# strukturag/libheif

Hardware: NVIDIA H100
Metric: megapixels/sec HEIC-grid decode->RGB (higher is better)
Workload: dtype u8

## Files before the change

libheif_b200/csrc/b200_hevc_entropy.cu:

```cuda
#include <cstdint>
#include <cstdlib>
namespace b200 { namespace syn {
__shared__ uint32_t s_kLps4[64];
__shared__ uint8_t s_kTransLps[64];
__shared__ uint8_t s_kNextState[256];
__shared__ unsigned long long s_kState[128];
__shared__ uint8_t s_kInitI[135];
__shared__ uint8_t s_kSigMap4[16];
__shared__ uint8_t s_kScanPos[3][16];
__shared__ uint8_t s_kScanInv[3][16];
__shared__ uint8_t s_kSbInv[4][3][64];
__shared__ uint8_t s_kSigCtx4[3][16];
__shared__ uint8_t s_kSigCtxN[3][4][16];
__shared__ uint8_t s_kChromaTab[4];
__shared__ uint8_t s_kScanX[4][3][64];
__shared__ uint8_t s_kScanY[4][3][64];
} }
#ifdef __CUDA_ARCH__
#define B200_T(name) s_##name
#endif
#include "b200_hevc.h"
static_assert(b200::syn::CTX_COUNT == 135, "s_kInitI above is sized for 135 context variables");

namespace b200 {

#ifndef B200_ENTROPY_WARPS
#define B200_ENTROPY_WARPS 4
#endif
constexpr int EWARPS = B200_ENTROPY_WARPS;

__device__ __forceinline__ unsigned e_ld_acquire(const unsigned* p) {
  unsigned v; asm volatile("ld.relaxed.gpu.global.u32 %0, [%1];" : "=r"(v) : "l"(p) : "memory"); return v;
}
__device__ __forceinline__ void e_st_release(unsigned* p, unsigned v) {
  asm volatile("st.release.gpu.global.u32 [%0], %1;" ::"l"(p), "r"(v) : "memory");
}
__device__ __forceinline__ unsigned e_poll(const unsigned* p) { return __shfl_sync(0xffffffffu, e_ld_acquire(p), 0); }
__device__ __forceinline__ bool lane0() { return syn::lane_id() == 0; }

#ifdef B200_ENTROPY_TRACE
constexpr int TRACE_CAP = 1 << 16;
__device__ unsigned long long g_trace[TRACE_CAP][2];
__device__ unsigned g_trace_sm[TRACE_CAP];
__device__ __forceinline__ unsigned long long e_globaltimer() { unsigned long long t; asm volatile("mov.u64 %0, %%globaltimer;" : "=l"(t)); return t; }
__device__ __forceinline__ unsigned e_smid() { unsigned s; asm volatile("mov.u32 %0, %%smid;" : "=r"(s)); return s; }
#endif

struct DevSync {
  unsigned* progress;
  unsigned* sub_done;
  unsigned* error_flag;
  unsigned* queue; unsigned* qtail; unsigned* deps;
  uint32_t dense_tu, dense_coef, dense_tu_cap, dense_coef_cap;
  uint64_t end_bit_position;
  __device__ static void spin_until(const unsigned* p, unsigned need, unsigned* error_flag) {
    if (e_poll(p) >= need) return;
    unsigned ns = 200, spins = 0;
    for (;;) {
      __nanosleep(ns); if (ns < 8000) ns <<= 1;
      if (e_poll(p) >= need) return;
      if ((++spins & 63u) != 0) continue;
      if (e_poll(error_flag)) return;
      if (spins > (1u << 23)) { if (lane0()) atomicExch(error_flag, 3u); return; }
    }
  }
  __device__ void wait_row(int row, int need) { spin_until(progress + row, (unsigned)need, error_flag); }
  __device__ void publish_row(int row, int done) { syn::warp_sync(); if (lane0()) e_st_release(progress + row, (unsigned)done); }
  __device__ void wait_substream(int idx) { spin_until(sub_done + idx, 1u, error_flag); }
  __device__ void finish_substream(int idx, int err) {
    syn::warp_sync();
    if (lane0()) {
      e_st_release(sub_done + idx, 1u);
      if (err) atomicExch(error_flag, (unsigned)err);
    }
  }
  __device__ void notify(int target) {
    if (target < 0) return;
    syn::warp_sync();
    if (lane0()) {
      __threadfence();
      if (atomicSub(deps + target, 1u) == 1u) { const unsigned s = atomicAdd(qtail, 1u); e_st_release(queue + s, (unsigned)target + 1u); }
    }
  }
};

#ifndef B200_ENTROPY_MIN_BLOCKS
#define B200_ENTROPY_MIN_BLOCKS 1
#endif
#ifndef B200_ENTROPY_MAX_BLOCKS_PER_SM
#define B200_ENTROPY_MAX_BLOCKS_PER_SM 0
#endif
template <class Cfg> constexpr int entropy_min_blocks() { return B200_ENTROPY_MIN_BLOCKS; }
template <> constexpr int entropy_min_blocks<syn::CfgCommon>() { return B200_ENTROPY_MIN_BLOCKS > 5 ? B200_ENTROPY_MIN_BLOCKS : 5; }
template <class Cfg>
__global__ void __launch_bounds__(EWARPS * 32, entropy_min_blocks<Cfg>()) hevc_entropy_kernel(const EntropyBatch b) {
  __shared__ __align__(8) syn::U2 s_ctx[EWARPS][syn::CTX_COUNT + syn::CTX_SCRATCH];
  __shared__ syn::DecoderT<Cfg> s_dec[EWARPS];
  __shared__ DevSync s_sync[EWARPS];
  for (int i = threadIdx.x; i < 64; i += blockDim.x) { syn::s_kLps4[i] = syn::d_kLps4[i]; syn::s_kTransLps[i] = syn::d_kTransLps[i]; }
  for (int i = threadIdx.x; i < syn::CTX_COUNT; i += blockDim.x) syn::s_kInitI[i] = syn::d_kInitI[i];
  for (int i = threadIdx.x; i < 256; i += blockDim.x) syn::s_kNextState[i] = syn::d_kNextState[i];
  for (int i = threadIdx.x; i < 128; i += blockDim.x) syn::s_kState[i] = syn::d_kState[i];
  for (int i = threadIdx.x; i < 16; i += blockDim.x) syn::s_kSigMap4[i] = syn::d_kSigMap4[i];
  for (int i = threadIdx.x; i < 48; i += blockDim.x) { (&syn::s_kScanPos[0][0])[i] = (&syn::d_kScanPos[0][0])[i]; (&syn::s_kScanInv[0][0])[i] = (&syn::d_kScanInv[0][0])[i]; (&syn::s_kSigCtx4[0][0])[i] = (&syn::d_kSigCtx4[0][0])[i]; }
  for (int i = threadIdx.x; i < 192; i += blockDim.x) (&syn::s_kSigCtxN[0][0][0])[i] = (&syn::d_kSigCtxN[0][0][0])[i];
  for (int i = threadIdx.x; i < 768; i += blockDim.x) (&syn::s_kSbInv[0][0][0])[i] = (&syn::d_kSbInv[0][0][0])[i];
  for (int i = threadIdx.x; i < 4; i += blockDim.x) syn::s_kChromaTab[i] = syn::d_kChromaTab[i];
  for (int i = threadIdx.x; i < 4 * 3 * 64; i += blockDim.x) { (&syn::s_kScanX[0][0][0])[i] = (&syn::d_kScanX[0][0][0])[i]; (&syn::s_kScanY[0][0][0])[i] = (&syn::d_kScanY[0][0][0])[i]; }
  __syncthreads();
  const int slot_w = threadIdx.x >> 5;
  const syn::CtxPtr ctx = (syn::CtxPtr)__cvta_generic_to_shared(s_ctx[slot_w]);
  for (;;) {
    unsigned slot = 0;
    if (lane0()) slot = atomicAdd(b.qhead, 1u);
    slot = __shfl_sync(0xffffffffu, slot, 0);
    if (slot >= (unsigned)b.nsubs) break;
    unsigned item = e_poll(b.queue + slot);
    if (!item) {
      unsigned ns = 500, spins = 0;
      for (;;) {
        __nanosleep(ns); if (ns < 16000) ns <<= 1;
        if ((item = e_poll(b.queue + slot)) != 0u) break;
        if ((++spins & 31u) != 0) continue;
        if (e_poll(b.error_flag)) return;
        if (spins > (1u << 22)) { if (lane0()) atomicExch(b.error_flag, 3u); return; }
      }
    }
#ifdef B200_ENTROPY_TRACE
    if (lane0() && item - 1u < (unsigned)TRACE_CAP) { g_trace[item - 1u][0] = e_globaltimer(); g_trace_sm[item - 1u] = e_smid(); }
#endif
    const syn::Substream& gs = b.subs[item - 1u];
    const EntropyPic& ep = b.pics[gs.pic];
    DevSync& sync = s_sync[slot_w];
    sync.progress = b.progress + ep.progress_base; sync.sub_done = b.sub_done + ep.sub_base; sync.error_flag = b.error_flag;
    sync.queue = b.queue; sync.qtail = b.qtail; sync.deps = b.deps;
    sync.dense_tu = sync.dense_coef = sync.dense_tu_cap = sync.dense_coef_cap = 0; sync.end_bit_position = 0;
    syn::run_substream<Cfg>(s_dec[slot_w], ep.sp, ep.pb, b.subs + ep.sub_base, (int)(item - 1u - ep.sub_base), ctx, sync);
#ifdef B200_ENTROPY_TRACE
    if (lane0() && item - 1u < (unsigned)TRACE_CAP) g_trace[item - 1u][1] = e_globaltimer();
#endif
  }
}

#ifdef B200_ENTROPY_TRACE
extern "C" int b200_debug_entropy_trace(unsigned long long* out, int n) {
  if (!out || n < 0 || n > TRACE_CAP) return set_error(B200_E_INVALID, "bad trace request");
  static unsigned long long t[TRACE_CAP][2]; static unsigned sm[TRACE_CAP];
  cudaError_t e = cudaDeviceSynchronize();
  if (e == cudaSuccess) e = cudaMemcpyFromSymbol(t, g_trace, sizeof t);
  if (e == cudaSuccess) e = cudaMemcpyFromSymbol(sm, g_trace_sm, sizeof sm);
  if (e != cudaSuccess) return set_error(B200_E_CUDA, "entropy trace: %s", cudaGetErrorString(e));
  for (int i = 0; i < n; i++) { out[3 * i] = t[i][0]; out[3 * i + 1] = t[i][1]; out[3 * i + 2] = sm[i]; }
  return B200_OK;
}
#endif
// ... 65 lines not shown
```

libheif_b200/csrc/b200_hevc_syntax.h:

```cpp
#pragma once
#include <cassert>
#include <cstdint>
#include <cstring>
#include "b200_hevc_types.h"

#if defined(__CUDA_ARCH__) && !defined(B200_SYNTAX_HOST_ONLY)
#define B200_SYN_DEVICE 1
#endif
#if defined(__CUDACC__) && !defined(B200_SYNTAX_HOST_ONLY)
#define B200_HDN __host__ __device__ __noinline__
#define B200_NOUNROLL _Pragma("unroll 1")
#define B200_HD __host__ __device__
#define B200_HDI __host__ __device__ __forceinline__
#define B200_TABLE(type, name, dims, ...) static const type h_##name dims = __VA_ARGS__; static __device__ const type d_##name dims = __VA_ARGS__;
#else
#define B200_HDN
#define B200_NOUNROLL
#define B200_HD
#define B200_HDI inline
#define B200_TABLE(type, name, dims, ...) static const type h_##name dims = __VA_ARGS__;
#endif
#if defined(B200_SYN_DEVICE) && !defined(B200_T)
#define B200_T(name) d_##name
#endif
// ... 84 lines not shown
#define B200_LANES_BEGIN() assert(__activemask() == 0xffffffffu)
#else
#define B200_LANES_BEGIN() ((void)0)
#endif
#define B200_LANE_FOR(k, n) B200_NOUNROLL for (int k = ::b200::syn::lane_id(); k < (n); k += 32)
#define B200_LANES_END() ::b200::syn::warp_sync()
#else
#define B200_LANES_BEGIN() ((void)0)
#define B200_LANE_FOR(k, n) B200_NOUNROLL for (int k = 0; k < (n); k++)
#define B200_LANES_END() ((void)0)
#endif

struct SeqParams {
  int32_t W, H, log2ctb, wctb, hctb, w4, w8, h8, chroma, bd;
  int32_t log2_min_cb, log2_min_tb, log2_max_tb, max_th_depth_intra;
  int32_t sao_enabled, transform_skip, cu_qp_delta, qg_log2, sign_hiding, wpp, sao_scale_luma, sao_scale_chroma;
  int32_t dense;
  int32_t tu_slots, coef_slots;
  int32_t pcm, pcm_bd_y, pcm_bd_c, pcm_shift_y, pcm_shift_c, log2_min_pcm, log2_max_pcm, pcm_lf_disabled;
  int32_t tq_bypass;
  int32_t tiles;
};

struct Substream {
  uint32_t pic;
  uint32_t byte_begin, byte_end;
  uint32_t ctb_begin, ctb_end;
  uint16_t tile_x0, tile_x1;
  uint32_t slice_addr_rs;
  int32_t slice_idx;
  int32_t slice_qp;
  uint8_t sao_luma, sao_chroma;
  uint8_t init_contexts;
  uint8_t last_of_segment;
  int32_t prev;
  int32_t wake_ctb2;
  int32_t wake_end;
  uint32_t deps;
};

struct PicBuffers {
  const uint8_t* rbsp; uint32_t rbsp_size;
  TuCmd* tus; CoefEntry* coefs; CtuInfo* ctus; const SliceInfo* slices;
  const uint16_t* ctu_slice;
  int8_t* qp8; uint8_t* edge8;
  uint8_t* ipm4;
  uint8_t* cd8;
  uint8_t* wpp_ctx;
  uint8_t* end_state;
};

B200_TABLE(uint8_t, kNextState, [256], {2,3,4,5,6,7,8,9,10,11,12,13,14,15,16,17,18,19,20,21,22,23,24,25,26,27,28,29,30,31,32,33,34,35,36,37,38,39,40,41,42,43,44,45,46,47,48,49,50,51,52,53,54,55,56,57,58,59,60,61,62,63,64,65,66,67,68,69,70,71,72,73,74,75,76,77,78,79,80,81,82,83,84,85,86,87,88,89,90,91,92,93,94,95,96,97,98,99,100,101,102,103,104,105,106,107,108,109,110,111,112,113,114,115,116,117,118,119,120,121,122,123,124,125,124,125,126,127,1,0,0,1,2,3,4,5,4,5,8,9,8,9,10,11,12,13,14,15,16,17,18,19,18,19,22,23,22,23,24,25,26,27,26,27,30,31,30,31,32,33,32,33,36,37,36,37,38,39,38,39,42,43,42,43,44,45,44,45,46,47,48,49,48,49,50,51,52,53,52,53,54,55,54,55,56,57,58,59,58,59,60,61,60,61,60,61,62,63,64,65,64,65,66,67,66,67,66,67,68,69,68,69,70,71,70,71,70,71,72,73,72,73,72,73,74,75,74,75,74,75,76,77,76,77,126,127})

B200_TABLE(uint64_t, kState, [128], {0x00000102f0d0b080ull,0x01000003f0d0b080ull,0x02000004e3c5a780ull,0x03000105e3c5a780ull,0x04000206d8bb9e80ull,0x05000307d8bb9e80ull,0x06000408cdb2967bull,0x07000509cdb2967bull,0x0800040ac3a98e74ull,0x0900050bc3a98e74ull,0x0a00080cb9a0876full,0x0b00090db9a0876full,0x0c00080eaf988069ull,0x0d00090faf988069ull,0x0e000a10a6907a64ull,0x0f000b11a6907a64ull,0x10000c129e89745full,0x11000d139e89745full,0x12000e1496826e5aull,0x13000f1596826e5aull,0x140010168e7b6855ull,0x150011178e7b6855ull,0x1600121887756351ull,0x1700131987756351ull,0x1800121a806f5e4dull,0x1900131b806f5e4dull,0x1a00161c7a695949ull,0x1b00171d7a695949ull,0x1c00161e74645545ull,0x1d00171f74645545ull,0x1e0018206e5f5042ull,0x1f0019216e5f5042ull,0x20001a22685a4c3eull,0x21001b23685a4c3eull,0x22001a246356483bull,0x23001b256356483bull,0x24001e265e514538ull,0x25001f275e514538ull,0x26001e28594d4135ull,0x27001f29594d4135ull,0x2800202a55493e33ull,0x2900212b55493e33ull,0x2a00202c50453b30ull,0x2b00212d50453b30ull,0x2c00242e4c42382eull,0x2d00252f4c42382eull,0x2e002430483f352bull,0x2f002531483f352bull,0x30002632453b3229ull,0x31002733453b3229ull,0x3200263441383027ull,0x3300273541383027ull,0x34002a363e362d25ull,0x35002b373e362d25ull,0x36002a383b332b23ull,0x37002b393b332b23ull,0x38002c3a38302921ull,0x39002d3b38302921ull,0x3a002c3c352e2720ull,0x3b002d3d352e2720ull,0x3c002e3e322b251eull,0x3d002f3f322b251eull,0x3e0030403029231dull,0x3f0031413029231dull,0x400030422d27211bull,0x410031432d27211bull,0x420032442b251f1aull,0x430033452b251f1aull,0x4400344629231e18ull,0x4500354729231e18ull,0x4600344827211c17ull,0x4700354927211c17ull,0x4800364a25201b16ull,0x4900374b25201b16ull,0x4a00364c231e1a15ull,0x4b00374d231e1a15ull,0x4c00384e211d1814ull,0x4d00394f211d1814ull,0x4e003a501f1b1713ull,0x4f003b511f1b1713ull,0x50003a521e1a1612ull,0x51003b531e1a1612ull,0x52003c541c191511ull,0x53003d551c191511ull,0x54003c561b171410ull,0x55003d571b171410ull,0x56003c581916130full,0x57003d591916130full,0x58003e5a1815120eull,0x59003f5b1815120eull,0x5a00405c1714110eull,0x5b00415d1714110eull,0x5c00405e1613100dull,0x5d00415f1613100dull,0x5e00426015120f0cull,0x5f00436115120f0cull,0x6000426214110e0cull,0x6100436314110e0cull,0x6200426413100e0bull,0x6300436513100e0bull,0x64004466120f0d0bull,0x65004567120f0d0bull,0x66004468110f0c0aull,0x67004569110f0c0aull,0x6800466a100e0c0aull,0x6900476b100e0c0aull,0x6a00466c0f0d0b09ull,0x6b00476d0f0d0b09ull,0x6c00466e0e0c0b09ull,0x6d00476f0e0c0b09ull,0x6e0048700e0c0a08ull,0x6f0049710e0c0a08ull,0x700048720d0b0908ull,0x710049730d0b0908ull,0x720048740c0b0907ull,0x730049750c0b0907ull,0x74004a760c0a0907ull,0x75004b770c0a0907ull,0x76004a780b0a0807ull,0x77004b790b0a0807ull,0x78004a7a0b090806ull,0x79004b7b0b090806ull,0x7a004c7c0a090706ull,0x7b004d7d0a090706ull,0x7c004c7c09080706ull,0x7d004d7d09080706ull,0x7e007e7e02020202ull,0x7f007f7f02020202ull})

struct CabacStream { const uint8_t* d; uint32_t size; };

struct Cabac {
  uint32_t val, range; int bits;
  uint32_t pos, next16;
  TabPtr state_tab;
  B200_HD static inline uint32_t fetch16(const CabacStream& st, uint32_t p) {
    const uint32_t q = p < st.size - 2 ? p : st.size - 2;
#ifdef B200_SYN_DEVICE
    return __byte_perm((uint32_t)__ldg(reinterpret_cast<const unsigned short*>(st.d + q)), 0, 0x4401);
#else
    return ((uint32_t)st.d[q] << 8) | st.d[q + 1];
#endif
  }
#ifdef B200_SYN_DEVICE
  static __device__ __noinline__ uint32_t fetch16_cold(const uint8_t* d, uint32_t q) { return __byte_perm((uint32_t)__ldg(reinterpret_cast<const unsigned short*>(d + q)), 0, 0x4401); }
#else
  static inline uint32_t fetch16_cold(const uint8_t* d, uint32_t q) { return ((uint32_t)d[q] << 8) | d[q + 1]; }
#endif
  B200_HD inline void start(const CabacStream& st, uint32_t start_byte) {
    if (start_byte & 1) {
      const uint32_t b0 = fetch16(st, start_byte - 1) & 0xffu, w1 = fetch16(st, start_byte + 1);
      val = ((b0 << 16) | w1) << 1; bits = 15; pos = start_byte + 3;
    } else {
      val = fetch16(st, start_byte) << 9; bits = 7; pos = start_byte + 2;
    }
    range = 510; next16 = fetch16(st, pos);
    state_tab = B200_TADDR(kState);
  }
  B200_HD inline uint64_t bit_position() const { return (uint64_t)pos * 8 - (uint32_t)bits; }
  B200_HD inline void shift(int n, const CabacStream& st) {
    val <<= n; bits -= n;
    if (bits < 0) { val |= next16 << (-bits); bits += 16; pos += 2; next16 = fetch16_cold(st.d, pos < st.size - 2 ? pos : st.size - 2); }
  }
  B200_HD inline int bin_e(const U2 e, CtxPtr c, const CabacStream& st, U2& ne) {
#ifdef B200_SYN_DEVICE
    uint32_t rlps; asm("prmt.b32 %0, 0, %1, %2;" : "=r"(rlps) : "r"(e.x), "r"(range >> 6));
#else
    const uint32_t rlps = (e.x >> (((range >> 6) & 3) * 8)) & 0xff;
#endif
    const uint32_t rmps = range - rlps, t = rmps << 16;
    const bool lps = val >= t;
    if (lps) val -= t;
    range = lps ? rlps : rmps;
    ne = tab_ld64(state_tab, (int)((lps ? e.y >> 8 : e.y) & 0xffu));
    ctx_st(c, ne);
#ifdef B200_SYN_DEVICE
    const int n = __clz((int)range) - 23;
#else
    const int n = __builtin_clz(range) - 23;
#endif
    range <<= n;
    shift(n, st);
    return (int)(((e.y >> 24) ^ (lps ? 1u : 0u)) & 1u);
  }
  B200_HD inline int bin(CtxPtr c, const CabacStream& st) { U2 ne; return bin_e(ctx_ld(c), c, st, ne); }
  B200_HD inline int bypass(const CabacStream& st) {
    shift(1, st);
    const uint32_t one = (val >> 16) >= range ? 1u : 0u;
    val -= one ? (range << 16) : 0u;
    return (int)one;
  }
  B200_HD inline unsigned bypass_bits(int k, const CabacStream& st) {
    unsigned out = 0;
    B200_NOUNROLL while (k > 0) {
      const int t = k > 7 ? 7 : k;
      shift(t, st);
      const uint32_t w = val >> 16;
#ifdef B200_SYN_DEVICE
      uint32_t q = (uint32_t)__float2int_rz(__fdividef((float)w, (float)range));
      int r = (int)w - (int)(q * range);
      if (r < 0) { q--; r += (int)range; } else if (r >= (int)range) { q++; r -= (int)range; }
      val = ((uint32_t)r << 16) | (val & 0xffffu);
#else
      const uint32_t q = w / range;
      val -= (q * range) << 16;
#endif
      out = (out << t) | (q & ((1u << t) - 1u)); k -= t;
    }
    return out;
  }
  B200_HD inline int terminate(const CabacStream& st) {
    range -= 2;
    if ((val >> 16) >= range) return 1;
    if (range < 256) { range <<= 1; shift(1, st); }
    return 0;
  }
};

B200_HDN inline void init_contexts(CtxPtr ctx, int slice_qp) {
  const int qp = clip3(0, 51, slice_qp);
  B200_LANES_BEGIN();
  B200_LANE_FOR(i, CTX_COUNT) {
    const int iv = B200_T(kInitI)[i], m = (iv >> 4) * 5 - 45, nn = ((iv & 15) << 3) - 16;
    const int pre = clip3(1, 126, ((m * qp) >> 4) + nn);
    const int mps = pre > 63, st = mps ? pre - 64 : 63 - pre;
    ctx_st(ctx_at(ctx, i), tab_ld64(B200_TADDR(kState), (st << 1) | mps));
  }
  B200_LANES_END();
}

B200_HDN inline void load_contexts(CtxPtr ctx, const uint8_t* st) {
  B200_LANES_BEGIN();
  B200_LANE_FOR(i, CTX_COUNT) ctx_st(ctx_at(ctx, i), tab_ld64(B200_TADDR(kState), (int)B200_LD_SHARED(st + i) & 127));
  B200_LANES_END();
}
B200_HDN inline void store_contexts(CtxPtr ctx, uint8_t* st) {
  B200_LANES_BEGIN();
  B200_LANE_FOR(i, CTX_COUNT) st[i] = (uint8_t)(ctx_ld(ctx_at(ctx, i)).y >> 24);
  B200_LANES_END();
}

enum { SYN_OK = 0, SYN_E_BITSTREAM = 1, SYN_E_OVERFLOW = 2 };

struct SaoRaw { int8_t type[3], band[3], eo[3]; int8_t off[3][4]; };

struct CfgRuntime { enum : int { chroma = -1, bd = -1, log2_min_cb = -1, log2_min_tb = -1, log2_max_tb = -1, transform_skip = -1, cu_qp_delta = -1, sign_hiding = -1, sao_enabled = -1, wpp = -1, dense = -1, pcm = -1, tq_bypass = -1, tiles = -1 }; };
struct CfgCommon { enum : int { chroma = 1, bd = 8, log2_min_cb = 3, log2_min_tb = 2, log2_max_tb = 5, transform_skip = 0, cu_qp_delta = 1, sign_hiding = 1, sao_enabled = 1, wpp = 1, dense = 0, pcm = 0, tq_bypass = 0, tiles = 0 }; };
B200_HD inline bool matches_common(const SeqParams& q) {
  return q.chroma == 1 && q.bd == 8 && q.log2_min_cb == 3 && q.log2_min_tb == 2 && q.log2_max_tb == 5 && !q.transform_skip && q.cu_qp_delta == 1 && q.sign_hiding == 1 &&
         q.sao_enabled == 1 && q.wpp == 1 && q.dense == 0 && !q.pcm && !q.tq_bypass && !q.tiles;
}
#define B200_SPC(f) ((int)Cfg::f >= 0 ? (int)Cfg::f : (int)sp->f)
#define B200_SPR(f) ((int)Cfg::f >= 0 ? (int)Cfg::f : (int)sp.f)

template <class Cfg>
struct DecoderT {
  const SeqParams* sp; PicBuffers pb; const Substream* ss;
  Cabac cabac; CabacStream stream; CtxPtr ctx;
  int is_dqp_coded, dqp_val, qpy_prev_qg, last_cu_qpy, first_qg, cur_qpy, err;
  int cu_bypass;
  uint32_t tu_n, coef_n, tu_cap, coef_cap;
  uint32_t ctb_tu0;
  int cur_ctb_x, cur_ctb_y;
  int ctb_x0, ctb_y0, left_ok, up_ok;
  int left_lf, up_lf;
  struct Cu { int x0, y0, log2cb, nxn, lmode[4], cmode; int cmodes[4]; };

  B200_HD inline bool avail(int x, int y) const { return x >= ctb_x0 ? (y >= ctb_y0 ? true : up_ok != 0) : left_ok != 0; }
  B200_HD inline int ld_cell(const uint8_t* p, int y) const { return y >= ctb_y0 ? (int)*p : (int)B200_LD_SHARED(p); }

  B200_HDN int dbin(int ci) { return cabac.bin(ctx_at(ctx, ci), stream); }
  B200_HDN int dbypass() { return cabac.bypass(stream); }
  B200_HDN unsigned dbits(int k) { return cabac.bypass_bits(k, stream); }

  B200_HDN void parse_sao(int rx, int ry, CtuInfo& ci) {
    const int addr = ry * sp->wctb + rx;
    B200_NOUNROLL for (int c = 0; c < 3; c++) { ci.sao[c].type = 0; ci.sao[c].band_or_class = 0; B200_NOUNROLL for (int k = 0; k < 4; k++) ci.sao[c].offset[k] = 0; }
    if (!ss->sao_luma && !ss->sao_chroma) return;
    int ml = 0, mu = 0;
    if (left_ok) ml = dbin(CTX_SAO_MERGE);
    if (up_ok && !ml) mu = dbin(CTX_SAO_MERGE);
    if (ml || mu) {
      const unsigned long long* o = reinterpret_cast<const unsigned long long*>(pb.ctus[ml ? addr - 1 : addr - sp->wctb].sao);
      unsigned long long* dsto = reinterpret_cast<unsigned long long*>(ci.sao);
      B200_NOUNROLL for (int c = 0; c < 3; c++) dsto[c] = B200_LD_SHARED(o + c);
      return;
    }
    B200_NOUNROLL for (int c = 0; c < (B200_SPC(chroma) ? 3 : 1); c++) {
      if ((c == 0 && !ss->sao_luma) || (c > 0 && !ss->sao_chroma)) continue;
      if (c < 2) { int t = 0; if (dbin(CTX_SAO_TYPE)) t = dbypass() ? 2 : 1; ci.sao[c].type = (uint8_t)t; } else ci.sao[2].type = ci.sao[1].type;
      if (!ci.sao[c].type) continue;
      const int cmax = (1 << (imin(B200_SPC(bd), 10) - 5)) - 1;
      int av[4];
      B200_NOUNROLL for (int i = 0; i < 4; i++) { int v = 0; B200_NOUNROLL while (v < cmax && dbypass()) v++; av[i] = v; }
      const int sc = c == 0 ? sp->sao_scale_luma : sp->sao_scale_chroma;
      if (ci.sao[c].type == 1) {
        B200_NOUNROLL for (int i = 0; i < 4; i++) if (av[i] && dbypass()) av[i] = -av[i];
        ci.sao[c].band_or_class = (uint8_t)dbits(5);
        B200_NOUNROLL for (int i = 0; i < 4; i++) ci.sao[c].offset[i] = (int8_t)clip3(-128, 127, av[i] * (1 << sc));
      } else {
        if (c < 2) ci.sao[c].band_or_class = (uint8_t)dbits(2); else ci.sao[2].band_or_class = ci.sao[1].band_or_class;
        ci.sao[c].offset[0] = (int8_t)clip3(-128, 127, av[0] << sc); ci.sao[c].offset[1] = (int8_t)clip3(-128, 127, av[1] << sc);
        ci.sao[c].offset[2] = (int8_t)clip3(-128, 127, -(av[2] << sc)); ci.sao[c].offset[3] = (int8_t)clip3(-128, 127, -(av[3] << sc));
      }
    }
  }

  B200_HDN void derive_qpy(int xcb, int ycb) {
    const int mask = (1 << sp->qg_log2) - 1, xqg = xcb & ~mask, yqg = ycb & ~mask, cm = ~((1 << sp->log2ctb) - 1);
    int qa = qpy_prev_qg, qb = qpy_prev_qg;
    if (avail(xqg - 1, yqg) && ((xqg - 1) & cm) == (xqg & cm)) qa = pb.qp8[(yqg >> 3) * sp->w8 + ((xqg - 1) >> 3)];
    if (avail(xqg, yqg - 1) && ((yqg - 1) & cm) == (yqg & cm)) qb = pb.qp8[((yqg - 1) >> 3) * sp->w8 + (xqg >> 3)];
    const int pred = (qa + qb + 1) >> 1, qbd = 6 * (B200_SPC(bd) - 8);
    cur_qpy = ((pred + dqp_val + 52 + 2 * qbd) % (52 + qbd)) - qbd;
  }

  B200_HDN int residual(int log2n, int c, int mode, int& tskip) {
    const int n = 1 << log2n;
    Cabac cb_ = cabac; const CtxPtr cx = ctx;
    const int bypass_cu = B200_SPC(tq_bypass) && cu_bypass;
    const int sign_hiding = B200_SPC(sign_hiding) && !bypass_cu;
    uint32_t cn = coef_n;
    tskip = 0;
    if (B200_SPC(transform_skip) && log2n == 2 && !bypass_cu) tskip = cb_.bin(ctx_at(cx, CTX_TSKIP + (c ? 1 : 0)), stream);
    const int cmax = (log2n << 1) - 1;
    int off, shift;
    if (c == 0) { off = 3 * (log2n - 2) + ((log2n - 1) >> 2); shift = (log2n + 1) >> 2; } else { off = 15; shift = log2n - 2; }
    int lx = 0, ly = 0;
    B200_NOUNROLL for (int xy = 0; xy < 2; xy++) {
      const CtxPtr lc = ctx_at(cx, (xy ? CTX_LAST_Y : CTX_LAST_X) + off);
      int l = 0;
      CtxPtr a_cur = lc; U2 e_cur = ctx_ld(a_cur);
      B200_NOUNROLL while (l < cmax) {
        const CtxPtr a_next = ctx_at(lc, (l + 1) >> shift);
        U2 e_next = ctx_ld(a_next), ne;
        const int b = cb_.bin_e(e_cur, a_cur, stream, ne);
        if (!b) break;
        if (a_next == a_cur) e_next = ne;
        a_cur = a_next; e_cur = e_next; l++;
      }
      if (xy) ly = l; else lx = l;
    }
    B200_NOUNROLL for (int xy = 0; xy < 2; xy++) {
      int l = xy ? ly : lx;
      if (l > 3) { const int nb = (l >> 1) - 1; l = (1 << nb) * (2 + (l & 1)) + (int)cb_.bypass_bits(nb, stream); }
      if (xy) ly = l; else lx = l;
    }
    int scan = 0;
    if (log2n == 2 || (log2n == 3 && (c == 0 || B200_SPC(chroma) == 3))) { if (mode >= 6 && mode <= 14) scan = 2; else if (mode >= 22 && mode <= 30) scan = 1; }
    if (scan == 2) { const int t = lx; lx = ly; ly = t; }
    if (lx >= n || ly >= n) { err = SYN_E_BITSTREAM; cabac = cb_; return 0; }
    const int l2sb = log2n - 2;
    const TabPtr sbx = B200_TADDR(kScanX) + 64 * (3 * l2sb + scan), sby = B200_TADDR(kScanY) + 64 * (3 * l2sb + scan), spos = B200_TADDR(kScanPos) + 16 * scan;
    const int last_sb = B200_T(kSbInv)[l2sb][scan][((ly >> 2) << 3) + (lx >> 2)];
    const int last_pos = B200_T(kScanInv)[scan][((ly & 3) << 2) + (lx & 3)];
    uint64_t csbf = 0;
    int carry = 1;
    const int sig_base = log2n == 2 ? CTX_SIG + (c ? 27 : 0) : (c == 0 ? CTX_SIG + (log2n == 3 ? (scan == 0 ? 9 : 15) : 21) : CTX_SIG + 27 + (log2n == 3 ? 9 : 12));
    B200_NOUNROLL for (int i = last_sb; i >= 0; i--) {
      const int xs = (int)tab_ld8(sbx, i), ys = (int)tab_ld8(sby, i);
      const int right = ((xs + 1) >> l2sb) == 0 ? (int)((csbf >> (ys * 8 + xs + 1)) & 1) : 0;
      const int below = ((ys + 1) >> l2sb) == 0 ? (int)((csbf >> ((ys + 1) * 8 + xs)) & 1) : 0;
      const bool is_last = csbf == 0;
      int infer_dc = 0;
      if (!is_last && i > 0) { if (!cb_.bin(ctx_at(cx, CTX_CSBF + ((right | below) ? 1 : 0) + (c ? 2 : 0)), stream)) continue; infer_dc = 1; }
      csbf |= 1ull << (ys * 8 + xs);
      const TabPtr tab = log2n == 2 ? B200_TADDR(kSigCtx4) + 16 * scan : B200_TADDR(kSigCtxN) + (64 * scan + 16 * (right | (below << 1)));
      const CtxPtr cbase = ctx_at(cx, sig_base + ((c == 0 && log2n > 2 && (xs | ys)) ? 3 : 0));
      unsigned sig = 0;
      int k = 15;
      if (is_last) { sig = 1u; k = last_pos - 1; }
      if (k >= 0) {
        const CtxPtr a0 = i == 0 ? ctx_at(cx, CTX_SIG + (c ? 27 : 0)) : ctx_at(cbase, (int)tab_ld8(tab, 0));
        CtxPtr a_cur = k > 0 ? ctx_at(cbase, (int)tab_ld8(tab, k)) : a0;
        U2 e_cur = ctx_ld(a_cur);
        B200_NOUNROLL for (; k > 0; k--) {
          const CtxPtr a_next = k > 1 ? ctx_at(cbase, (int)tab_ld8(tab, k - 1)) : a0;
          U2 e_next = ctx_ld(a_next), ne;
          sig = (sig << 1) | (unsigned)cb_.bin_e(e_cur, a_cur, stream, ne);
          if (a_next == a_cur) e_next = ne;
          a_cur = a_next; e_cur = e_next;
        }
        if (infer_dc && !sig) sig = 1u;
        else { U2 ne; sig = (sig << 1) | (unsigned)cb_.bin_e(e_cur, a_cur, stream, ne); }
      }
      if (!sig) continue;
      unsigned g1 = 0;
      int g1ctx = 1, g2 = 0;
      int ctx_set = (i == 0 || c > 0) ? 0 : 2;
      if (carry == 0) ctx_set++;
      const int last_sig = hi_bit(sig), first_sig = lo_bit(sig);
      { unsigned m = sig; const CtxPtr gbase = ctx_at(cx, CTX_GT1 + ctx_set * 4 + (c ? 16 : 0));
        B200_NOUNROLL for (int ng1 = 0; m && ng1 < 8; ng1++) {
          const int kk = hi_bit(m); m ^= 1u << kk;
          if (cb_.bin(ctx_at(gbase, imin(3, g1ctx)), stream)) { g1 |= 1u << kk; g1ctx = 0; } else if (g1ctx > 0) g1ctx++;
        } }
      carry = g1ctx;
      const int last_g1 = g1 ? hi_bit(g1) : -1;
      const bool hidden = sign_hiding && (last_sig - first_sig > 3);
      if (last_g1 >= 0) g2 = cb_.bin(ctx_at(cx, CTX_GT2 + ctx_set + (c ? 4 : 0)), stream);
      const int nsign = pop_count(sig) - (hidden ? 1 : 0);
      const unsigned signs = cb_.bypass_bits(nsign, stream);
#ifdef B200_SYN_DEVICE
      int nsig = 0, sum = 0, rice = 0;
      const uint32_t lv = ctx_at(cx, CTX_COUNT);
      B200_NOUNROLL for (unsigned m = sig; m; nsig++) {
        const int kk = hi_bit(m); m ^= 1u << kk;
        const int base = 1 + (int)((g1 >> kk) & 1) + (kk == last_g1 ? g2 : 0);
        int a = base;
        if (base == ((nsig < 8) ? ((kk == last_g1) ? 3 : 2) : 1)) {
          int pre = 0; B200_NOUNROLL while (pre < 32 && cb_.bypass(stream)) pre++;
          if (pre > 20) { err = SYN_E_BITSTREAM; cabac = cb_; const int count = (int)(cn - coef_n); coef_n = cn; return count; }
          const int rem = (pre <= 3 ? (pre << rice) : (((1 << (pre - 3)) + 3 - 1) << rice)) + (int)cb_.bypass_bits(pre <= 3 ? rice : pre - 3 + rice, stream);
          a = base + rem;
          if (a > 3 * (1 << rice)) rice = imin(rice + 1, 4);
        }
        sum += a;
        asm volatile("st.shared.u32 [%0], %1;" ::"r"(lv + 4u * (uint32_t)kk), "r"(a));
      }
      if (cn + (uint32_t)nsig > coef_cap) { err = SYN_E_OVERFLOW; cabac = cb_; const int count = (int)(cn - coef_n); coef_n = cn; return count; }
      B200_LANES_BEGIN();
      { const int k = lane_id();
        if (k < 16 && ((sig >> k) & 1u)) {
          int a; asm volatile("ld.shared.u32 %0, [%1];" : "=r"(a) : "r"(lv + 4u * (uint32_t)k));
          const int above = pop_count(sig >> k >> 1);
          const int neg = (hidden && k == first_sig) ? (sum & 1) : (int)((signs >> (nsign - 1 - above)) & 1u);
          const int p = (int)tab_ld8(spos, k);
          CoefEntry e; e.pos = (uint16_t)((((ys << 2) + (p >> 2)) << log2n) + (xs << 2) + (p & 3)); e.level = (int16_t)clip3(-32768, 32767, neg ? -a : a);
          pb.coefs[cn + (uint32_t)above] = e;
        } }
      B200_LANES_END();
      cn += (uint32_t)nsig;
#else
      int nsig = 0, sum = 0, rice = 0, sidx = nsign;
// ... 446 lines not shown
```

Measured before the change: 4079.

## Encode CABAC next-state as absolute shared-memory address in context entries

The CABAC state table grows to 256 entries, indexed by state and LPS bit, and each context entry now stores a precomputed shared-memory address of its successor entry, with the shared base folded in at kernel start. A state transition becomes a single load at e.y plus an offset, which removes the shift/mask indexing and the per-decoder state_tab pointer. The last-significant-position and sig-coeff loops also drop the speculative prefetch of the next context and reload it after each bin, which lengthens the serial dependency chain. Context save/restore and init are adjusted to the new encoding.

```diff
diff --git a/libheif_b200/csrc/b200_hevc_entropy.cu b/libheif_b200/csrc/b200_hevc_entropy.cu
--- a/libheif_b200/csrc/b200_hevc_entropy.cu
+++ b/libheif_b200/csrc/b200_hevc_entropy.cu
@@ -4,7 +4,7 @@
 __shared__ uint32_t s_kLps4[64];
 __shared__ uint8_t s_kTransLps[64];
 __shared__ uint8_t s_kNextState[256];
-__shared__ unsigned long long s_kState[128];
+__shared__ __align__(16) unsigned long long s_kState[256];
 __shared__ uint8_t s_kInitI[135];
 __shared__ uint8_t s_kSigMap4[16];
 __shared__ uint8_t s_kScanPos[3][16];
@@ -100,7 +100,9 @@
   for (int i = threadIdx.x; i < 64; i += blockDim.x) { syn::s_kLps4[i] = syn::d_kLps4[i]; syn::s_kTransLps[i] = syn::d_kTransLps[i]; }
   for (int i = threadIdx.x; i < syn::CTX_COUNT; i += blockDim.x) syn::s_kInitI[i] = syn::d_kInitI[i];
   for (int i = threadIdx.x; i < 256; i += blockDim.x) syn::s_kNextState[i] = syn::d_kNextState[i];
-  for (int i = threadIdx.x; i < 128; i += blockDim.x) syn::s_kState[i] = syn::d_kState[i];
+  {
+    const unsigned long long base = (unsigned long long)syn::state_base() << 32;
+    for (int i = threadIdx.x; i < 256; i += blockDim.x) syn::s_kState[i] = syn::d_kState[i] + base; }
   for (int i = threadIdx.x; i < 16; i += blockDim.x) syn::s_kSigMap4[i] = syn::d_kSigMap4[i];
   for (int i = threadIdx.x; i < 48; i += blockDim.x) { (&syn::s_kScanPos[0][0])[i] = (&syn::d_kScanPos[0][0])[i]; (&syn::s_kScanInv[0][0])[i] = (&syn::d_kScanInv[0][0])[i]; (&syn::s_kSigCtx4[0][0])[i] = (&syn::d_kSigCtx4[0][0])[i]; }
   for (int i = threadIdx.x; i < 192; i += blockDim.x) (&syn::s_kSigCtxN[0][0][0])[i] = (&syn::d_kSigCtxN[0][0][0])[i];
diff --git a/libheif_b200/csrc/b200_hevc_syntax.h b/libheif_b200/csrc/b200_hevc_syntax.h
--- a/libheif_b200/csrc/b200_hevc_syntax.h
+++ b/libheif_b200/csrc/b200_hevc_syntax.h
@@ -160,14 +160,23 @@
 
 B200_TABLE(uint8_t, kNextState, [256], {2,3,4,5,6,7,8,9,10,11,12,13,14,15,16,17,18,19,20,21,22,23,24,25,26,27,28,29,30,31,32,33,34,35,36,37,38,39,40,41,42,43,44,45,46,47,48,49,50,51,52,53,54,55,56,57,58,59,60,61,62,63,64,65,66,67,68,69,70,71,72,73,74,75,76,77,78,79,80,81,82,83,84,85,86,87,88,89,90,91,92,93,94,95,96,97,98,99,100,101,102,103,104,105,106,107,108,109,110,111,112,113,114,115,116,117,118,119,120,121,122,123,124,125,124,125,126,127,1,0,0,1,2,3,4,5,4,5,8,9,8,9,10,11,12,13,14,15,16,17,18,19,18,19,22,23,22,23,24,25,26,27,26,27,30,31,30,31,32,33,32,33,36,37,36,37,38,39,38,39,42,43,42,43,44,45,44,45,46,47,48,49,48,49,50,51,52,53,52,53,54,55,54,55,56,57,58,59,58,59,60,61,60,61,60,61,62,63,64,65,64,65,66,67,66,67,66,67,68,69,68,69,70,71,70,71,70,71,72,73,72,73,72,73,74,75,74,75,74,75,76,77,76,77,126,127})
 
-B200_TABLE(uint64_t, kState, [128], {0x00000102f0d0b080ull,0x01000003f0d0b080ull,0x02000004e3c5a780ull,0x03000105e3c5a780ull,0x04000206d8bb9e80ull,0x05000307d8bb9e80ull,0x06000408cdb2967bull,0x07000509cdb2967bull,0x0800040ac3a98e74ull,0x0900050bc3a98e74ull,0x0a00080cb9a0876full,0x0b00090db9a0876full,0x0c00080eaf988069ull,0x0d00090faf988069ull,0x0e000a10a6907a64ull,0x0f000b11a6907a64ull,0x10000c129e89745full,0x11000d139e89745full,0x12000e1496826e5aull,0x13000f1596826e5aull,0x140010168e7b6855ull,0x150011178e7b6855ull,0x1600121887756351ull,0x1700131987756351ull,0x1800121a806f5e4dull,0x1900131b806f5e4dull,0x1a00161c7a695949ull,0x1b00171d7a695949ull,0x1c00161e74645545ull,0x1d00171f74645545ull,0x1e0018206e5f5042ull,0x1f0019216e5f5042ull,0x20001a22685a4c3eull,0x21001b23685a4c3eull,0x22001a246356483bull,0x23001b256356483bull,0x24001e265e514538ull,0x25001f275e514538ull,0x26001e28594d4135ull,0x27001f29594d4135ull,0x2800202a55493e33ull,0x2900212b55493e33ull,0x2a00202c50453b30ull,0x2b00212d50453b30ull,0x2c00242e4c42382eull,0x2d00252f4c42382eull,0x2e002430483f352bull,0x2f002531483f352bull,0x30002632453b3229ull,0x31002733453b3229ull,0x3200263441383027ull,0x3300273541383027ull,0x34002a363e362d25ull,0x35002b373e362d25ull,0x36002a383b332b23ull,0x37002b393b332b23ull,0x38002c3a38302921ull,0x39002d3b38302921ull,0x3a002c3c352e2720ull,0x3b002d3d352e2720ull,0x3c002e3e322b251eull,0x3d002f3f322b251eull,0x3e0030403029231dull,0x3f0031413029231dull,0x400030422d27211bull,0x410031432d27211bull,0x420032442b251f1aull,0x430033452b251f1aull,0x4400344629231e18ull,0x4500354729231e18ull,0x4600344827211c17ull,0x4700354927211c17ull,0x4800364a25201b16ull,0x4900374b25201b16ull,0x4a00364c231e1a15ull,0x4b00374d231e1a15ull,0x4c00384e211d1814ull,0x4d00394f211d1814ull,0x4e003a501f1b1713ull,0x4f003b511f1b1713ull,0x50003a521e1a1612ull,0x51003b531e1a1612ull,0x52003c541c191511ull,0x53003d551c191511ull,0x54003c561b171410ull,0x55003d571b171410ull,0x56003c581916130full,0x57003d591916130full,0x58003e5a1815120eull,0x59003f5b1815120eull,0x5a00405c1714110eull,0x5b00415d1714110eull,0x5c00405e1613100dull,0x5d00415f1613100dull,0x5e00426015120f0cull,0x5f00436115120f0cull,0x6000426214110e0cull,0x6100436314110e0cull,0x6200426413100e0bull,0x6300436513100e0bull,0x64004466120f0d0bull,0x65004567120f0d0bull,0x66004468110f0c0aull,0x67004569110f0c0aull,0x6800466a100e0c0aull,0x6900476b100e0c0aull,0x6a00466c0f0d0b09ull,0x6b00476d0f0d0b09ull,0x6c00466e0e0c0b09ull,0x6d00476f0e0c0b09ull,0x6e0048700e0c0a08ull,0x6f0049710e0c0a08ull,0x700048720d0b0908ull,0x710049730d0b0908ull,0x720048740c0b0907ull,0x730049750c0b0907ull,0x74004a760c0a0907ull,0x75004b770c0a0907ull,0x76004a780b0a0807ull,0x77004b790b0a0807ull,0x78004a7a0b090806ull,0x79004b7b0b090806ull,0x7a004c7c0a090706ull,0x7b004d7d0a090706ull,0x7c004c7c09080706ull,0x7d004d7d09080706ull,0x7e007e7e02020202ull,0x7f007f7f02020202ull})
+B200_TABLE(uint64_t, kState, [256], {0x00000020e3c5a780ull,0x00000010f0d0b080ull,0x00000030e3c5a780ull,0x00000000f0d0b080ull,0x00000040d8bb9e80ull,0x00000000f0d0b080ull,0x00000050d8bb9e80ull,0x00000010f0d0b080ull,0x00000060cdb2967bull,0x00000020e3c5a780ull,0x00000070cdb2967bull,0x00000030e3c5a780ull,0x00000080c3a98e74ull,0x00000040d8bb9e80ull,0x00000090c3a98e74ull,0x00000050d8bb9e80ull,0x000000a0b9a0876full,0x00000040d8bb9e80ull,0x000000b0b9a0876full,0x00000050d8bb9e80ull,0x000000c0af988069ull,0x00000080c3a98e74ull,0x000000d0af988069ull,0x00000090c3a98e74ull,0x000000e0a6907a64ull,0x00000080c3a98e74ull,0x000000f0a6907a64ull,0x00000090c3a98e74ull,0x000001009e89745full,0x000000a0b9a0876full,0x000001109e89745full,0x000000b0b9a0876full,0x0000012096826e5aull,0x000000c0af988069ull,0x0000013096826e5aull,0x000000d0af988069ull,0x000001408e7b6855ull,0x000000e0a6907a64ull,0x000001508e7b6855ull,0x000000f0a6907a64ull,0x0000016087756351ull,0x000001009e89745full,0x0000017087756351ull,0x000001109e89745full,0x00000180806f5e4dull,0x0000012096826e5aull,0x00000190806f5e4dull,0x0000013096826e5aull,0x000001a07a695949ull,0x0000012096826e5aull,0x000001b07a695949ull,0x0000013096826e5aull,0x000001c074645545ull,0x0000016087756351ull,0x000001d074645545ull,0x0000017087756351ull,0x000001e06e5f5042ull,0x0000016087756351ull,0x000001f06e5f5042ull,0x0000017087756351ull,0x00000200685a4c3eull,0x00000180806f5e4dull,0x00000210685a4c3eull,0x00000190806f5e4dull,0x000002206356483bull,0x000001a07a695949ull,0x000002306356483bull,0x000001b07a695949ull,0x000002405e514538ull,0x000001a07a695949ull,0x000002505e514538ull,0x000001b07a695949ull,0x00000260594d4135ull,0x000001e06e5f5042ull,0x00000270594d4135ull,0x000001f06e5f5042ull,0x0000028055493e33ull,0x000001e06e5f5042ull,0x0000029055493e33ull,0x000001f06e5f5042ull,0x000002a050453b30ull,0x00000200685a4c3eull,0x000002b050453b30ull,0x00000210685a4c3eull,0x000002c04c42382eull,0x00000200685a4c3eull,0x000002d04c42382eull,0x00000210685a4c3eull,0x000002e0483f352bull,0x000002405e514538ull,0x000002f0483f352bull,0x000002505e514538ull,0x00000300453b3229ull,0x000002405e514538ull,0x00000310453b3229ull,0x000002505e514538ull,0x0000032041383027ull,0x00000260594d4135ull,0x0000033041383027ull,0x00000270594d4135ull,0x000003403e362d25ull,0x00000260594d4135ull,0x000003503e362d25ull,0x00000270594d4135ull,0x000003603b332b23ull,0x000002a050453b30ull,0x000003703b332b23ull,0x000002b050453b30ull,0x0000038038302921ull,0x000002a050453b30ull,0x0000039038302921ull,0x000002b050453b30ull,0x000003a0352e2720ull,0x000002c04c42382eull,0x000003b0352e2720ull,0x000002d04c42382eull,0x000003c0322b251eull,0x000002c04c42382eull,0x000003d0322b251eull,0x000002d04c42382eull,0x000003e03029231dull,0x000002e0483f352bull,0x000003f03029231dull,0x000002f0483f352bull,0x000004002d27211bull,0x00000300453b3229ull,0x000004102d27211bull,0x00000310453b3229ull,0x000004202b251f1aull,0x00000300453b3229ull,0x000004302b251f1aull,0x00000310453b3229ull,0x0000044029231e18ull,0x0000032041383027ull,0x0000045029231e18ull,0x0000033041383027ull,0x0000046027211c17ull,0x000003403e362d25ull,0x0000047027211c17ull,0x000003503e362d25ull,0x0000048025201b16ull,0x000003403e362d25ull,0x0000049025201b16ull,0x000003503e362d25ull,0x000004a0231e1a15ull,0x000003603b332b23ull,0x000004b0231e1a15ull,0x000003703b332b23ull,0x000004c0211d1814ull,0x000003603b332b23ull,0x000004d0211d1814ull,0x000003703b332b23ull,0x000004e01f1b1713ull,0x0000038038302921ull,0x000004f01f1b1713ull,0x0000039038302921ull,0x000005001e1a1612ull,0x000003a0352e2720ull,0x000005101e1a1612ull,0x000003b0352e2720ull,0x000005201c191511ull,0x000003a0352e2720ull,0x000005301c191511ull,0x000003b0352e2720ull,0x000005401b171410ull,0x000003c0322b251eull,0x000005501b171410ull,0x000003d0322b251eull,0x000005601916130full,0x000003c0322b251eull,0x000005701916130full,0x000003d0322b251eull,0x000005801815120eull,0x000003c0322b251eull,0x000005901815120eull,0x000003d0322b251eull,0x000005a01714110eull,0x000003e03029231dull,0x000005b01714110eull,0x000003f03029231dull,0x000005c01613100dull,0x000004002d27211bull,0x000005d01613100dull,0x000004102d27211bull,0x000005e015120f0cull,0x000004002d27211bull,0x000005f015120f0cull,0x000004102d27211bull,0x0000060014110e0cull,0x000004202b251f1aull,0x0000061014110e0cull,0x000004302b251f1aull,0x0000062013100e0bull,0x000004202b251f1aull,0x0000063013100e0bull,0x000004302b251f1aull,0x00000640120f0d0bull,0x000004202b251f1aull,0x00000650120f0d0bull,0x000004302b251f1aull,0x00000660110f0c0aull,0x0000044029231e18ull,0x00000670110f0c0aull,0x0000045029231e18ull,0x00000680100e0c0aull,0x0000044029231e18ull,0x00000690100e0c0aull,0x0000045029231e18ull,0x000006a00f0d0b09ull,0x0000046027211c17ull,0x000006b00f0d0b09ull,0x0000047027211c17ull,0x000006c00e0c0b09ull,0x0000046027211c17ull,0x000006d00e0c0b09ull,0x0000047027211c17ull,0x000006e00e0c0a08ull,0x0000046027211c17ull,0x000006f00e0c0a08ull,0x0000047027211c17ull,0x000007000d0b0908ull,0x0000048025201b16ull,0x000007100d0b0908ull,0x0000049025201b16ull,0x000007200c0b0907ull,0x0000048025201b16ull,0x000007300c0b0907ull,0x0000049025201b16ull,0x000007400c0a0907ull,0x0000048025201b16ull,0x000007500c0a0907ull,0x0000049025201b16ull,0x000007600b0a0807ull,0x000004a0231e1a15ull,0x000007700b0a0807ull,0x000004b0231e1a15ull,0x000007800b090806ull,0x000004a0231e1a15ull,0x000007900b090806ull,0x000004b0231e1a15ull,0x000007a00a090706ull,0x000004a0231e1a15ull,0x000007b00a090706ull,0x000004b0231e1a15ull,0x000007c009080706ull,0x000004c0211d1814ull,0x000007d009080706ull,0x000004d0211d1814ull,0x000007c009080706ull,0x000004c0211d1814ull,0x000007d009080706ull,0x000004d0211d1814ull,0x000007e002020202ull,0x000007e002020202ull,0x000007f002020202ull,0x000007f002020202ull})
+
+#ifdef B200_SYN_DEVICE
+__device__ __forceinline__ U2 state_ld(uint32_t h) { return tab_ld64(h, 0); }
+__device__ __forceinline__ uint32_t state_base() { return B200_TADDR(kState); }
+#else
+inline U2 state_ld(uint32_t h) { return tab_ld64(B200_TADDR(kState), (int)(h >> 3)); }
+inline uint32_t state_base() { return 0; }
+#endif
+B200_HD inline U2 state_entry(int b) { return U2{tab_ld32(B200_TADDR(kLps4), b >> 1), state_base() + 16u * (uint32_t)b}; }
+B200_HD inline uint32_t state_byte(U2 e) { return (e.y - state_base()) >> 4; }
 
 struct CabacStream { const uint8_t* d; uint32_t size; };
 
 struct Cabac {
   uint32_t val, range; int bits;
   uint32_t pos, next16;
-  TabPtr state_tab;
   B200_HD static inline uint32_t fetch16(const CabacStream& st, uint32_t p) {
     const uint32_t q = p < st.size - 2 ? p : st.size - 2;
 #ifdef B200_SYN_DEVICE
@@ -189,7 +198,6 @@
       val = fetch16(st, start_byte) << 9; bits = 7; pos = start_byte + 2;
     }
     range = 510; next16 = fetch16(st, pos);
-    state_tab = B200_TADDR(kState);
   }
   B200_HD inline uint64_t bit_position() const { return (uint64_t)pos * 8 - (uint32_t)bits; }
   B200_HD inline void shift(int n, const CabacStream& st) {
@@ -206,7 +214,8 @@
     const bool lps = val >= t;
     if (lps) val -= t;
     range = lps ? rlps : rmps;
-    ne = tab_ld64(state_tab, (int)((lps ? e.y >> 8 : e.y) & 0xffu));
+    const uint32_t lb = lps ? 1u : 0u;
+    ne = state_ld(e.y + (lb << 3));
     ctx_st(c, ne);
 #ifdef B200_SYN_DEVICE
     const int n = __clz((int)range) - 23;
@@ -215,7 +224,7 @@
 #endif
     range <<= n;
     shift(n, st);
-    return (int)(((e.y >> 24) ^ (lps ? 1u : 0u)) & 1u);
+    return (int)(((e.y >> 4) ^ lb) & 1u);
   }
   B200_HD inline int bin(CtxPtr c, const CabacStream& st) { U2 ne; return bin_e(ctx_ld(c), c, st, ne); }
   B200_HD inline int bypass(const CabacStream& st) {
@@ -258,19 +267,19 @@
     const int iv = B200_T(kInitI)[i], m = (iv >> 4) * 5 - 45, nn = ((iv & 15) << 3) - 16;
     const int pre = clip3(1, 126, ((m * qp) >> 4) + nn);
     const int mps = pre > 63, st = mps ? pre - 64 : 63 - pre;
-    ctx_st(ctx_at(ctx, i), tab_ld64(B200_TADDR(kState), (st << 1) | mps));
+    ctx_st(ctx_at(ctx, i), state_entry((st << 1) | mps));
   }
   B200_LANES_END();
 }
 
 B200_HDN inline void load_contexts(CtxPtr ctx, const uint8_t* st) {
   B200_LANES_BEGIN();
-  B200_LANE_FOR(i, CTX_COUNT) ctx_st(ctx_at(ctx, i), tab_ld64(B200_TADDR(kState), (int)B200_LD_SHARED(st + i) & 127));
+  B200_LANE_FOR(i, CTX_COUNT) ctx_st(ctx_at(ctx, i), state_entry((int)B200_LD_SHARED(st + i) & 127));
   B200_LANES_END();
 }
 B200_HDN inline void store_contexts(CtxPtr ctx, uint8_t* st) {
   B200_LANES_BEGIN();
-  B200_LANE_FOR(i, CTX_COUNT) st[i] = (uint8_t)(ctx_ld(ctx_at(ctx, i)).y >> 24);
+  B200_LANE_FOR(i, CTX_COUNT) st[i] = (uint8_t)state_byte(ctx_ld(ctx_at(ctx, i)));
   B200_LANES_END();
 }
 
@@ -364,14 +373,11 @@
     B200_NOUNROLL for (int xy = 0; xy < 2; xy++) {
       const CtxPtr lc = ctx_at(cx, (xy ? CTX_LAST_Y : CTX_LAST_X) + off);
       int l = 0;
-      CtxPtr a_cur = lc; U2 e_cur = ctx_ld(a_cur);
+      CtxPtr a_cur = lc;
       B200_NOUNROLL while (l < cmax) {
-        const CtxPtr a_next = ctx_at(lc, (l + 1) >> shift);
-        U2 e_next = ctx_ld(a_next), ne;
-        const int b = cb_.bin_e(e_cur, a_cur, stream, ne);
-        if (!b) break;
-        if (a_next == a_cur) e_next = ne;
-        a_cur = a_next; e_cur = e_next; l++;
+        U2 ne;
+        if (!cb_.bin_e(ctx_ld(a_cur), a_cur, stream, ne)) break;
+        l++; a_cur = ctx_at(lc, l >> shift);
       }
       if (xy) ly = l; else lx = l;
     }
@@ -410,10 +416,9 @@
         U2 e_cur = ctx_ld(a_cur);
         B200_NOUNROLL for (; k > 0; k--) {
           const CtxPtr a_next = k > 1 ? ctx_at(cbase, (int)tab_ld8(tab, k - 1)) : a0;
-          U2 e_next = ctx_ld(a_next), ne;
+          U2 ne;
           sig = (sig << 1) | (unsigned)cb_.bin_e(e_cur, a_cur, stream, ne);
-          if (a_next == a_cur) e_next = ne;
-          a_cur = a_next; e_cur = e_next;
+          a_cur = a_next; e_cur = ctx_ld(a_cur);
         }
         if (infer_dc && !sig) sig = 1u;
         else { U2 ne; sig = (sig << 1) | (unsigned)cb_.bin_e(e_cur, a_cur, stream, ne); }
```

Measured after the change: 4222, median of 6. 3.5% higher.
